# LingmaFuture/PRCV2025REID

Hardware: AMD Instinct MI355X
Metric: multimodal instances/sec (PxK, 5-modality) at 1/2/4/8 GPU; eval queries/sec (higher is better)
Workload: dtype bf16; 1 GPU; P=16,K=4 per GPU, vis/nir/sk/cp 224x224 + text (T<=77), CLIP ViT-B/16 + text tower random-init, MER-LoRA r=8, masks all-on, 400 ids, SDM+CE, fwd+bwd+grad sanitise/clip+AdamW (reference default trainable set); P=16, K=4, global_batch=64, lora_rank=8, accum_steps=1, parallelism=dp1

## Files before the change

### include/reid_hip.h

```cpp
#ifndef REID_HIP_H
#define REID_HIP_H

#include <stdint.h>

#ifdef __cplusplus
extern "C" {
#endif

typedef enum {
    REID_OK = 0,
    REID_ERR_ARG = -1,
    REID_ERR_LAUNCH = -2,
    REID_ERR_DEVICE = -3
} reid_status;

typedef enum { REID_BF16 = 0, REID_F32 = 1, REID_F16 = 2 } reid_dtype;

typedef enum {
    REID_ACT_NONE = 0,
    REID_ACT_GELU_ERF = 1,
    REID_ACT_QUICK_GELU = 2,
    REID_ACT_RELU = 3,
    REID_ACT_DGELU_ERF = 4,
    REID_ACT_DQUICK_GELU = 5,
// ... 45 lines not shown
                       const int32_t* row_index, const float* gamma, const float* mean, const float* rstd,
                       const void* dres, void* dx, int32_t dx_dtype, void* dx_bf16, int32_t lddx,
                       float* dgamma, float* dbeta, int32_t rows, int32_t cols,
                       const float* bf16_row_scale, int32_t rows_per_img, int32_t* overflow, void* stream);

int reid_patch_im2col(const float* images, void* patches, int32_t n_img, int32_t H, int32_t W,
                      int32_t patch, int32_t cin, void* stream);
int reid_cls_rows(const float* cls, const float* pos0, float* x, int32_t ldx, int32_t n_img,
                  int32_t tokens, int32_t cols, void* stream);

int reid_attn_fwd(const void* qkv, int32_t ld, const uint8_t* key_mask, void* out, int32_t ldo, float* lse,
                  int32_t n_seq, int32_t S, int32_t heads, int32_t causal, int32_t q_tiles, void* stream);
int reid_attn_bwd(const void* qkv, int32_t ld, const uint8_t* key_mask, const void* out, const void* dout,
                  int32_t ldo, const float* lse, void* dqkv, int32_t lddqkv, float* delta_ws,
                  int32_t n_seq, int32_t S, int32_t heads, int32_t causal, int32_t q_tiles, void* stream);

int reid_cast_f32_bf16(const float* src, void* dst, int64_t n, void* stream);
int reid_cast_bf16_f32(const void* src, float* dst, int64_t n, void* stream);
int reid_pack_bf16_table(const float* src, void* dst_bf16, const int64_t* table, int32_t n_entries, void* stream);
int reid_lora_bwd_fused(const void* dY, int32_t lddy, const void* T, int32_t ldt, const void* BT, int32_t ldbt, void* U, int32_t ldu,
                        float* dB, int32_t lddb, const int32_t* img_mod, int32_t rows_per_img, int32_t mask_r, int32_t M, int32_t N,
                        int32_t Rp, float scale, float* u_partial, int32_t u_mode, void* stream);
int reid_lora_da_fused(const void* X, int32_t ldx, const void* U, int32_t ldu, float* dA, int32_t ldda, const int32_t* img_mod,
                       int32_t rows_per_img, int32_t mask_r, int32_t M, int32_t K, int32_t Rp, int32_t n_groups, void* stream);

int reid_merge_lora_table(const int64_t* table, int32_t n_entries, int32_t max_tiles, const float* arena, void* weff,
                          int32_t Rp, int32_t r, int32_t nmod, float scaling, void* stream);
int reid_gather_rows_f32(const float* src, int32_t lds, const int32_t* index, float* dst, int32_t ldd,
                         int32_t rows, int32_t cols, void* stream);
int reid_embed_tokens(const float* tok, const float* pos, const int64_t* ids, float* out, int32_t B, int32_t T, int32_t D,
// ... 136 lines not shown
```

### prcv2025reid_amd/_lib.py

```python
import ctypes as C
import os

import torch

_HERE = os.path.dirname(os.path.abspath(__file__))
LIB_PATHS = {'bf16': os.path.join(_HERE, 'csrc', 'libreid_hip.so'), 'f16': os.path.join(_HERE, 'csrc', 'libreid_hip_f16.so')}
if os.environ.get('REID_LIB_BF16'):
    LIB_PATHS['bf16'] = os.environ['REID_LIB_BF16']
LIB_PATH = LIB_PATHS['bf16']
T16_DTYPES = {'bf16': torch.bfloat16, 'f16': torch.float16}
_flavor = os.environ.get('REID_T16', 'bf16')


def set_flavor(name: str):
    global _flavor
    if name not in LIB_PATHS:
        raise ValueError(f'unknown 16-bit flavor {name!r}')
    _flavor = name


def flavor() -> str:
    return _flavor


# ... 28 lines not shown
SIGNATURES = {
    'reid_last_error': (_S, []),
    'reid_version': (_I, []),
    'reid_flavor': (_I, []),
    'reid_check_device': (_I, [_I]),
    'reid_set_knob': (_I, [_S, _I]),
    'reid_mer_gemm': (_I, [_GEMM, _P]),
    'reid_gemm_tn': (_I, [_P, _P, _P, _I, _I, _I, _I, _I, _I, _F, _F, _P]),
    'reid_layernorm_fwd': (_I, [_P, _I, _P, _P, _P, _P, _P, _I, _P, _P, _I, _I, _F, _P]),
    'reid_add_layernorm_fwd': (_I, [_P, _I, _P, _I, _I, _P, _I, _P, _I, _P, _P, _P, _I, _P, _P, _I, _I, _F, _P]),
    'reid_layernorm_bwd': (_I, [_P, _I, _I, _P, _I, _P, _P, _P, _P, _P, _P, _I, _P, _I, _P, _P, _I, _I, _P, _I, _P, _P]),
    'reid_patch_im2col': (_I, [_P, _P, _I, _I, _I, _I, _I, _P]),
    'reid_cls_rows': (_I, [_P, _P, _P, _I, _I, _I, _I, _P]),
    'reid_attn_fwd': (_I, [_P, _I, _P, _P, _I, _P, _I, _I, _I, _I, _I, _P]),
    'reid_attn_bwd': (_I, [_P, _I, _P, _P, _P, _I, _P, _P, _I, _P, _I, _I, _I, _I, _I, _P]),
    'reid_cast_f32_bf16': (_I, [_P, _P, _I64, _P]),
    'reid_cast_bf16_f32': (_I, [_P, _P, _I64, _P]),
    'reid_pack_bf16_table': (_I, [_P, _P, _P, _I, _P]),
    'reid_lora_bwd_fused': (_I, [_P, _I, _P, _I, _P, _I, _P, _I, _P, _I, _P, _I, _I, _I, _I, _I, _F, _P, _I, _P]),
    'reid_lora_da_fused': (_I, [_P, _I, _P, _I, _P, _I, _P, _I, _I, _I, _I, _I, _I, _P]),
    'reid_merge_lora_table': (_I, [_P, _I, _I, _P, _P, _I, _I, _I, _F, _P]),
    'reid_gather_rows_f32': (_I, [_P, _I, _P, _P, _I, _I, _I, _P]),
    'reid_embed_tokens': (_I, [_P, _P, _P, _P, _I, _I, _I, _I, _P]),
    'reid_scatter_add_rows_f32': (_I, [_P, _I, _P, _P, _I, _I, _I, _I, _P]),
    'reid_bnneck_stats': (_I, [_P, _I, _I, _I, _P, _P, _P]),
    'reid_bnneck_fwd': (_I, [_P, _I, _P, _P, _P, _P, _P, _P, _F, _I, _P, _P, _I, _P, _P, _P, _I, _I, _F, _F, _F, _P]),
    'reid_bnneck_bwd_p1': (_I, [_P, _I, _P, _I, _P, _P, _P, _P, _P, _P, _P, _P, _I, _I, _F, _P]),
    'reid_bnneck_bwd_p2': (_I, [_P, _P, _I, _P, _P, _P, _P, _P, _F, _I, _P, _I, _I, _I, _P]),
    'reid_ce_ls_fwd': (_I, [_P, _I, _P, _P, _I, _I, _F, _P, _P, _P]),
    'reid_ce_ls_bwd': (_I, [_P, _I, _P, _P, _I, _I, _F, _P, _P, _I, _P]),
# ... 120 lines not shown
```

### prcv2025reid_amd/csrc/attention.hip

```cpp
#include "lds_tile.h"
#include <stdlib.h>

namespace {

using namespace ldstile;

constexpr float LOG2E = 1.4426950408889634f;

template <int NT>
__device__ __forceinline__ void stage_head(const bf16_t* __restrict__ base, int ld, int S, char* lds, int wave, int lane,
                                           int row_limit = 1 << 30) {
#pragma unroll
    for (int i = 0; i < 4; ++i) {
        const int rblk = (i * NT + wave) * 8;
        if (rblk >= row_limit) continue;
        stage_rows8(lds, rblk, lane, [&](int row, int c) { return base + (size_t)(row < S ? row : S - 1) * ld + c * 8; });
    }
}

__device__ __forceinline__ bf16x8 row_frag(const char* img, int row0, int kchunk, int lane) {
    const int row = row0 + (lane & 31);
    return *(const bf16x8*)(img + row * 128 + (swz(row, kchunk + (lane >> 5)) << 4));
}

// ... 42 lines not shown
__device__ __forceinline__ bf16x8 pack8(const f32x16& a, int s) {
    bf16x8 r;
#pragma unroll
    for (int j = 0; j < 8; ++j) r[j] = (short)f32_to_bf16(a[8 * s + j]);
    return r;
}

__device__ __forceinline__ int acc_row(int reg, int lane) { return (reg & 3) + 8 * (reg >> 2) + 4 * (lane >> 5); }

struct AttnParams {
    const bf16_t* qkv; int ld; const uint8_t* key_mask;
    bf16_t* out; int ldo; float* lse;
    const bf16_t* dout; bf16_t* dqkv; int lddqkv; float* delta;
    int n_seq, S, heads, causal;
    int q_tiles;
};

__device__ __forceinline__ void store_tile_row16(bf16_t* row, bool ok, const f32x16& t, float scale, int lane) {
#pragma unroll
    for (int j = 0; j < 2; ++j) {
        const int a = 8 * j, b = 8 * j + 4;
        const auto r0 = __builtin_amdgcn_permlane32_swap(pack_bf16x2(t[a] * scale, t[a + 1] * scale),
                                                         pack_bf16x2(t[b] * scale, t[b + 1] * scale), false, false);
        const auto r1 = __builtin_amdgcn_permlane32_swap(pack_bf16x2(t[a + 2] * scale, t[a + 3] * scale),
                                                         pack_bf16x2(t[b + 2] * scale, t[b + 3] * scale), false, false);
        if (ok) *(uint4*)(row + 8 * (2 * j + (lane >> 5))) = uint4{r0[0], r1[0], r0[1], r1[1]};
    }
}


template <int NT, bool TWO_PASS>
__global__ __launch_bounds__(NT * 64, TWO_PASS ? 4 : 1) void attn_fwd_kernel(const AttnParams p) {
    REID_T16_ENTER();
    extern __shared__ __attribute__((aligned(16))) char smem[];
    char* Ks = smem;
    char* Vs = smem + NT * 32 * 128;
    const int tid = threadIdx.x, lane = tid & 63;
    const int wave = __builtin_amdgcn_readfirstlane(tid >> 6);
    const int seq = blockIdx.x / p.heads, head = blockIdx.x % p.heads;
    const int d = p.heads * 64;
    const bf16_t* qb = p.qkv + (size_t)seq * p.S * p.ld + head * 64;
    stage_head<NT>(qb + d, p.ld, p.S, Ks, wave, lane);
    const int q0 = wave * 32;
    const int qi = q0 + (lane & 31);
    const int qrow = qi < p.S ? qi : p.S - 1;
    bf16x8 qf[4];
#pragma unroll
    for (int ks = 0; ks < 4; ++ks) qf[ks] = gfrag(qb, p.ld, qrow, 2 * ks, lane);
    stage_head<NT>(qb + 2 * d, p.ld, p.S, Vs, wave, lane);
    __syncthreads();
    if (q0 >= p.S || (p.q_tiles > 0 && wave >= p.q_tiles)) return;

    const FragOff fo = make_frag_off(lane);
    const uint8_t* km = p.key_mask ? p.key_mask + (size_t)seq * p.S : nullptr;
    const int h4 = 4 * (lane >> 5);
    const bool general = km != nullptr || p.causal;
    auto score_tile = [&](int kt) -> f32x16 {
        f32x16 t;
#pragma unroll
// ... 302 lines not shown
    char* Ds = smem + 2 * IMG;
    float* rowc = (float*)(Ds + NT * 32 * DS_ROW);
    const int tid = threadIdx.x, lane = tid & 63;
    const int wave = __builtin_amdgcn_readfirstlane(tid >> 6);
    const int seq = blockIdx.x / p.heads, head = blockIdx.x % p.heads;
    const int d = p.heads * 64;
    const bf16_t* qb = p.qkv + (size_t)seq * p.S * p.ld + head * 64;
    const bf16_t* gb = p.dout + (size_t)seq * p.S * p.ldo + head * 64;
    const bf16_t* ob = p.out + (size_t)seq * p.S * p.ldo + head * 64;
    const int nq = p.q_tiles > 0 ? (p.q_tiles < NT ? p.q_tiles : NT) : NT;
    const int q_rows = nq * 32;
    const int t0 = wave * 32;
    const int ti = t0 + (lane & 31);
    const int trow = ti < p.S ? ti : p.S - 1;
    const bool own_q = wave < nq;
    bf16x8 kf[4], vf[4];
#pragma unroll
    for (int ks = 0; ks < 4; ++ks) {
        kf[ks] = gfrag(qb + d, p.ld, trow, 2 * ks, lane);
        vf[ks] = gfrag(qb + 2 * d, p.ld, trow, 2 * ks, lane);
    }
    stage_head<NT>(qb, p.ld, p.S, Qs, wave, lane, q_rows);
    stage_head<NT>(gb, p.ldo, p.S, Gs, wave, lane, q_rows);
    bf16x8 of[4];
#pragma unroll
    for (int ks = 0; ks < 4; ++ks) of[ks] = gfrag(ob, p.ldo, trow, 2 * ks, lane);
    const size_t so = ((size_t)seq * p.heads + head) * p.S + trow;
    const float lse_v = p.lse[so];
    const FragOff fo = make_frag_off(lane);
    __syncthreads();
// ... 164 lines not shown
    (void)hipMemcpyToSymbol(HIP_SYMBOL(g_attn_bwd_trace), &ptr, sizeof(ptr));
}
#endif

#define DISPATCH_NT(nt, fn, ...)                \
    switch (nt) {                               \
        case 1: return fn<1>(__VA_ARGS__);      \
        case 2: return fn<2>(__VA_ARGS__);      \
        case 3: return fn<3>(__VA_ARGS__);      \
        case 4: return fn<4>(__VA_ARGS__);      \
        case 5: return fn<5>(__VA_ARGS__);      \
        case 6: return fn<6>(__VA_ARGS__);      \
        default: return fn<7>(__VA_ARGS__);     \
    }

extern "C" int reid_attn_fwd(const void* qkv, int32_t ld, const uint8_t* key_mask, void* out, int32_t ldo, float* lse,
                             int32_t n_seq, int32_t S, int32_t heads, int32_t causal, int32_t q_tiles, void* stream) {
    int rc = check_common("reid_attn_fwd", qkv, ld, n_seq, S, heads);
    if (rc) return rc;
    REID_CHECK_ARG(out && ldo >= heads * 64 && ldo % 4 == 0, "reid_attn_fwd: out/ldo");
    AttnParams p{(const bf16_t*)qkv, ld, key_mask, (bf16_t*)out, ldo, lse, nullptr, nullptr, 0, nullptr, n_seq, S, heads, causal, q_tiles};
    DISPATCH_NT((S + 31) / 32, launch_fwd, p, (hipStream_t)stream)
}

extern "C" int reid_attn_bwd(const void* qkv, int32_t ld, const uint8_t* key_mask, const void* out, const void* dout,
                             int32_t ldo, const float* lse, void* dqkv, int32_t lddqkv, float* delta_ws, int32_t n_seq,
                             int32_t S, int32_t heads, int32_t causal, int32_t q_tiles, void* stream) {
    int rc = check_common("reid_attn_bwd", qkv, ld, n_seq, S, heads);
    if (rc) return rc;
    REID_CHECK_ARG(out && dout && lse && dqkv && delta_ws, "reid_attn_bwd: null pointer");
    REID_CHECK_ARG(ldo >= heads * 64 && ldo % 8 == 0 && lddqkv >= 3 * heads * 64 && lddqkv % 4 == 0, "reid_attn_bwd: ldo/lddqkv");
    AttnParams p{(const bf16_t*)qkv, ld, key_mask, (bf16_t*)out, ldo, (float*)lse, (const bf16_t*)dout, (bf16_t*)dqkv, lddqkv,
                 delta_ws, n_seq, S, heads, causal, q_tiles};
    DISPATCH_NT((S + 31) / 32, launch_bwd, p, (hipStream_t)stream)
}
```

### prcv2025reid_amd/csrc/lora.hip

```cpp
#include "lds_tile.h"
#include <type_traits>

namespace {
using namespace ldstile;

constexpr int MT = 64;

__global__ __launch_bounds__(256) void merge_lora_kernel(const int64_t* __restrict__ table, const float* __restrict__ arena,
                                                         bf16_t* __restrict__ weff, int Rp, int r, int nmod, float s) {
    REID_T16_ENTER();
    const int64_t* e = table + (size_t)blockIdx.y * 8;
    const int N = (int)e[5], K = (int)e[6], G = (int)e[7];
    const int tiles_k = K / MT;
    if ((int)blockIdx.x >= (N / MT) * tiles_k) return;
    const float* __restrict__ W = (const float*)e[0];
    const float* __restrict__ A = arena + e[1];
    const float* __restrict__ B = arena + e[2];
    bf16_t* dst = weff + e[3];
    bf16_t* dstT = e[4] >= 0 ? weff + e[4] : nullptr;
    const int n0 = ((int)blockIdx.x / tiles_k) * MT, k0 = ((int)blockIdx.x % tiles_k) * MT;
    const int g = n0 / (N / G);
    const int R = nmod * r;
    __shared__ __attribute__((aligned(16))) float sW[MT][MT + 4];
    __shared__ __attribute__((aligned(16))) float sA[MT][MT + 4];
// ... 196 lines not shown

namespace image {
constexpr int N = fused::N, R = 32;
constexpr int ROW_BYTES = N * 2;
constexpr int IMG_BYTES = R * ROW_BYTES;
constexpr int NBUF = 3;
template <int RP> struct BwdGeo {
    static constexpr int T_BYTES = RP == 32 ? R * RP * 2 : R * 32;
    static constexpr int BUF_BYTES = IMG_BYTES + T_BYTES;
    static constexpr int USTAGE_BYTES = R * RP * 2;
    static constexpr int LDS_BYTES = NBUF * BUF_BYTES + USTAGE_BYTES;
};
using fused::Params;

constexpr int MAX_SPAN = 8;
__device__ __forceinline__ uint64_t span_mods(const int32_t* img_mod, int i0, int cnt) {
    uint64_t m = 0;
#pragma unroll
    for (int i = 0; i < MAX_SPAN; ++i) m |= (uint64_t)(img_mod[i0 + (i < cnt ? i : cnt - 1)] & 255) << (8 * i);
    return m;
}
__device__ __forceinline__ int span_mod(uint64_t mods, int i) { return (int)(mods >> (8 * i)) & 255; }

__device__ __forceinline__ bf16x8 tr_frag_swz(const char* img, int col0, int lane) {
    const int l16 = lane & 15, fq = lane >> 4;
    const int q = l16 >> 2, pp = l16 & 3;
    const int col = col0 + 4 * pp;
    const int r0 = 4 * fq + q, r1 = r0 + 16;
    const char* a0 = img + r0 * ROW_BYTES + (swz512(r0, col >> 3) << 4) + (col & 7) * 2;
    const char* a1 = img + r1 * ROW_BYTES + (swz512(r1, col >> 3) << 4) + (col & 7) * 2;
    return tr_join(tr_read(a0), tr_read(a1));
}

template <class P, class Run>
__device__ __forceinline__ void for_each_run(const P& p, Run run) {
    const int i0 = blockIdx.x * p.span, cnt = min(p.n_img - i0, p.span);
    const uint64_t mods = span_mods(p.img_mod, i0, cnt);
    for (int a = 0; a < cnt;) {
        const int mu = span_mod(mods, a);
        int b = a + 1;
        while (b < cnt && span_mod(mods, b) == mu) ++b;
        const int rbeg = (i0 + a) * p.rows_per_img;
        const int rend = min(p.M, (i0 + b) * p.rows_per_img);
        if (rbeg >= rend) break;
        a = b;
        run(rbeg, rend, mu, a < cnt);
    }
}

__device__ __forceinline__ void dma_tile(const bf16_t* const& src, const int& ld, const int& r0, const int& rend, const int& w, const int& lane, const uint32_t& base) {
#pragma unroll
    for (int j = 0; j < 6; ++j) {
        const int qd = w * 6 + j;
        const int g = qd * 64 + lane;
// ... 20 lines not shown
template <class Issue>
__device__ __forceinline__ int ring_refill(int t, int steps, int buf, Issue& issue) {
    const int nb = buf == 0 ? NBUF - 1 : buf - 1;
    if (t + 2 < steps) issue(t + 2, nb);
    return buf + 1 == NBUF ? 0 : buf + 1;
}

__global__ __launch_bounds__(256) void u_finish_kernel(const float* __restrict__ Up, bf16_t* __restrict__ U, int ldu, const int32_t* __restrict__ img_mod,
                                                       int rows_per_img, int mask_r, float scale, int M, int Rp) {
    REID_T16_ENTER();
    const int i = blockIdx.x * 256 + threadIdx.x;
    const int h = Rp >> 1;
    const int m = i / h, c = (i - m * h) * 2;
    if (m >= M) return;
    const int mu = img_mod[m / rows_per_img];
    const float a = Up[(size_t)m * Rp + c], b = Up[(size_t)m * Rp + c + 1];
    *(uint32_t*)(U + (size_t)m * ldu + c) = pack_bf16x2(c / mask_r == mu ? a * scale : 0.f, (c + 1) / mask_r == mu ? b * scale : 0.f);
}

template <int RP>
__device__ __forceinline__ void lora_bwd_image_run(const Params& p, char* smem, const int rbeg, const int rend, const int mu) {
    constexpr int BUF_BYTES = BwdGeo<RP>::BUF_BYTES;
    int tid = threadIdx.x;
    asm volatile("" : "+v"(tid));
    const int lane = tid & 63;
    const int w = __builtin_amdgcn_readfirstlane(tid >> 6);
    const int l16 = lane & 15, fq = lane >> 4;
    const int w0 = (mu * p.mask_r) & ~15;
    const int c_lo = mu * p.mask_r - w0, c_hi = c_lo + p.mask_r;
    const int steps = (rend - rbeg + R - 1) / R;
// ... 143 lines not shown
    __syncthreads();
    {
        const int rr = p.mask_r, total = N * rr;
        for (int idx = ftid; idx < total; idx += 512) {
            const int col = idx / rr, j = idx - col * rr;
            atomicAdd(p.dB + (size_t)col * p.lddb + mu * rr + j, fl[col * 16 + c_lo + j]);
        }
    }
}

template <int RP>
__global__ __launch_bounds__(512, 2) void lora_bwd_image_kernel(const Params p) {
    REID_T16_ENTER();
    static_assert(RP == 32 || RP == 64, "adapter columns");
    extern __shared__ __attribute__((aligned(16))) char smem[];
    for_each_run(p, [=](int rbeg, int rend, int mu, bool more) { lora_bwd_image_run<RP>(p, smem, rbeg, rend, mu); if (more) __syncthreads(); });
}

struct DaParams {
    const bf16_t* X; const bf16_t* U; float* dA;
    const int32_t* img_mod;
    int ldx, ldu, ldda, rows_per_img, mask_r, M, Rp, span, n_img;
};
template <int G>
__device__ __forceinline__ void lora_da_image_run(const DaParams& p, char* smem, const int rbeg, const int rend, const int mu, const bool more) {
    constexpr int UB = 4096;
    constexpr int BUF = IMG_BYTES + UB;
    const int tid = threadIdx.x, lane = tid & 63;
    const int w = __builtin_amdgcn_readfirstlane(tid >> 6);
    const int l16 = lane & 15, fq = lane >> 4;
    const int cblk = blockIdx.y;
// ... 47 lines not shown
    for (int e = 0; e < 4; ++e) {
        const int c = 4 * fq + e;
        if (c < c_lo || c >= c_hi) continue;
#pragma unroll
        for (int g = 0; g < G; ++g)
#pragma unroll
            for (int i = 0; i < 6; ++i)
                atomicAdd(p.dA + (size_t)(g * p.Rp + w0 + c) * p.ldda + (size_t)cblk * N + w * 96 + i * 16 + l16, acc[g][i][e]);
    }
}

template <int G>
__global__ __launch_bounds__(512, 2) void lora_da_image_kernel(const DaParams p) {
    REID_T16_ENTER();
    extern __shared__ __attribute__((aligned(16))) char smem[];
    for_each_run(p, [=](int rbeg, int rend, int mu, bool more) { lora_da_image_run<G>(p, smem, rbeg, rend, mu, more); });
}
}

}

static int lora_span(int n_img) {
    const int k = reid_knob(KNOB_LORA_SPAN);
    if (k == 1 || k == 2 || k == 4 || k == 8) return k;
    return n_img >= reid_num_cus() ? 4 : 1;
}

static bool lora_image_shape(int rows_per_img, int mask_r) { return rows_per_img >= image::R && mask_r <= 16 && 16 % mask_r == 0; }

extern "C" int reid_lora_bwd_fused(const void* dY, int32_t lddy, const void* T, int32_t ldt, const void* BT, int32_t ldbt, void* U,
                                   int32_t ldu, float* dB, int32_t lddb, const int32_t* img_mod, int32_t rows_per_img, int32_t mask_r,
// ... 76 lines not shown
```

### prcv2025reid_amd/engine.py

```python
from types import SimpleNamespace
from typing import Dict, List, Optional, Tuple

import math
import os

import torch

from . import _lib, ops

LIN = ('qkv', 'out', 'fc1', 'fc2')
REF_LIN = {'attn.q_proj': ('qkv', 0), 'attn.k_proj': ('qkv', 1), 'attn.v_proj': ('qkv', 2), 'attn.out_proj': ('out', 0),
           'mlp.fc1': ('fc1', 0), 'mlp.fc2': ('fc2', 0)}


def round_up(a, b):
    return (a + b - 1) // b * b


def grad_scale(amax):
    return torch.exp2(torch.floor(torch.log2(512.0 / amax))).clamp(2.0 ** -20, 2.0 ** 40)


class DenseGrads:

# ... 78 lines not shown
        e = self.ent[(l, nm)]
        n_out = e['N'] // e['G']
        return self.view_B(arena, l, nm)[g * n_out:(g + 1) * n_out, mu * r:(mu + 1) * r]

    def weff(self, arena, l, nm, transposed=False):
        e = self.ent[(l, nm)]
        N, K = e['N'], e['K']
        return self._view(arena, e['wET' if transposed else 'wE'], (self.nmod, K, N) if transposed else (self.nmod, N, K))

    def pk(self, pack, l, nm, which):
        e = self.ent[(l, nm)]
        G, K, N, Rp = e['G'], e['K'], e['N'], self.Rp
        return self._view(pack, e['p' + which], {'A': (G * Rp, K), 'AT': (K, G * Rp), 'B': (N, Rp), 'BT': (Rp, N)}[which])


class Engine:

    def __init__(self, arch: dict, P: Dict[str, torch.Tensor], lora_arena: torch.Tensor, device, layout: Optional[LoraLayout] = None):
        self.arch = arch
        self.P = P
        self.lora_arena = lora_arena
        self.dev = device
        self.lay = layout if layout is not None else LoraLayout(arch)
        self.S = (arch['image_size'] // arch['patch_size']) ** 2 + 1
        self.scaling = arch['lora_alpha'] / arch['lora_rank']
        self.flavor = _lib.flavor()
        self.loss_scaling = self.flavor == 'f16'
        self.dx_half = os.environ.get('REID_DX_HALF', '1') != '0'
        self.dx_overflow = torch.zeros(1, dtype=torch.int32, device=device)
        self._dense_ver = None
        self._lora_ver = None
        self._lora_pack = None
        self._weff = None
        self._merge_table = None
        self._table = None
        self._pack = self._text = self._side = None
        self._pack_event = None
        self._text_pending = None
        self._consts = {}
        self._rng = torch.Generator(device=device)
        self._rng.manual_seed(777)
        self.pending_drop_scales = None
        self._text_packed = None
        self.overlap_tn = os.environ.get('REID_TN_STREAM', '1') != '0'
# ... 109 lines not shown
        dv = sum(p._version for k, p in self.P.items() if k.startswith('clip_encoder.') and p is not self.lora_arena)
        tt = self.text_trains()
        dense_changed = dv != self._dense_ver or tt != self._text_packed
        if dense_changed:
            self.pack_dense(); self._dense_ver = dv; self._text_packed = tt
        lv = self.lora_arena._version
        if lv != self._lora_ver or dense_changed:
            self.pack_lora(); self._lora_ver = lv

    def drop_path_scales(self, n_img: int, rate: float):
        L = self.arch['vision_layers']
        keep = self._const(('dp_keep', L, float(rate)),
                           lambda: torch.tensor([1.0 - rate * l / max(1, L - 1) for l in range(L)], dtype=torch.float32))
        u = torch.rand(L, 2, n_img, device=self.dev, generator=self._rng)
        sc = torch.floor(u + keep.view(L, 1, 1)) / keep.view(L, 1, 1)
        return [(None, None) if rate * l / max(1, L - 1) <= 0.0 else (sc[l, 0], sc[l, 1]) for l in range(L)]

    def vision_forward(self, groups: List[Tuple[int, torch.Tensor]], save: bool, drop_scales=None):
        a, P, W, lay = self.arch, self.P, self.W, self.lay
        dev = self.dev
        S, d, ff, Rp = self.S, lay.d, lay.ff, lay.Rp
        heads = a['vision_heads']
        n_img = sum(g[1].shape[0] for g in groups)
        M = n_img * S
        ce = 'clip_encoder.'
        mods = []
        for mu, img in groups:
            mods += [mu] * img.shape[0]
        img_mod = self._const(('img_mod', tuple(mods)), lambda: torch.tensor(mods, dtype=torch.int32))
        f32, b16 = self._kw()
        x = torch.empty(M, d, **f32)
# ... 55 lines not shown

        L = a['vision_layers']
        nxt = None
        for l in range(L):
            lp = f'{ce}vision_layers.{l}.'
            if nxt is None:
                h = new('h', (M, d), b16); mean1 = new('m1', (M,), f32); rstd1 = new('r1', (M,), f32)
                ops.layernorm_fwd(x, P[lp + 'ln1.weight'], P[lp + 'ln1.bias'], y_bf16=h, mean=mean1, rstd=rstd1)
            else:
                h, mean1, rstd1 = nxt
                nxt = None
            qkv = new('qkv', (M, 3 * d), b16)
            ops.gemm(h, we(l, 'qkv'), qkv, bias=W[('v', l, 'bqkv')], row_groups=full.rg)
            last = l == L - 1
            o = new('o', (M, d), b16); lse = new('lse', (n_img, heads, S), f32)
            ops.attn_fwd(qkv, o, lse, n_img, S, heads, q_tiles=1 if last else 0)
            sa, sm_ = (None, None) if drop_scales is None else drop_scales[l]
            rows = cls if last else full
            xin, oin = (x.index_select(0, idxl), o.index_select(0, idxl)) if last else (x, o)
            Mr, rpi, rg = rows.M, rows.rpi, rows.rg
            xm = new('xm', (Mr, d), f32)
            h2 = new('h2', (Mr, d), b16); mean2 = new('m2', (Mr,), f32); rstd2 = new('r2', (Mr,), f32)
            if not last:
                yb = buf.get('yb')
                if yb is None:
                    yb = buf['yb'] = torch.empty(M, d, dtype=torch.float16, device=dev)
                ops.gemm(oin, we(l, 'out'), yb, bias=P[lp + 'attn.out_proj.shared_linear.bias'], row_groups=rg)
                ops.add_layernorm_fwd(xin, yb, xm, P[lp + 'ln2.weight'], P[lp + 'ln2.bias'], h2, mean2, rstd2, row_scale=sa, rows_per_img=rpi)
            else:
                ops.gemm(oin, we(l, 'out'), xm, bias=P[lp + 'attn.out_proj.shared_linear.bias'], R=xin, row_scale=sa, rows_per_img=rpi,
                         row_groups=rg)
                ops.layernorm_fwd(xm, P[lp + 'ln2.weight'], P[lp + 'ln2.bias'], y_bf16=h2, mean=mean2, rstd=rstd2)
# ... 14 lines not shown
                nxt = (new('h' + str((l + 1) & 1), (M, d), b16), new('m1' + str((l + 1) & 1), (M,), f32), new('r1' + str((l + 1) & 1), (M,), f32))
                ops.add_layernorm_fwd(xm, yb, xn, P[np_ + 'ln1.weight'], P[np_ + 'ln1.bias'], nxt[0], nxt[1], nxt[2], row_scale=sm_,
                                      rows_per_img=rpi)
            else:
                ops.gemm(g, we(l, 'fc2'), xn, bias=P[lp + 'mlp.fc2.shared_linear.bias'], R=xm, row_scale=sm_, rows_per_img=rpi,
                         row_groups=rg)
            if save:
                saved.append(dict(x=x, h=h, mean1=mean1, rstd1=rstd1, T=T, qkv=qkv, o=o, lse=lse, To=To, xm=xm, h2=h2,
                                  mean2=mean2, rstd2=rstd2, T1=T1, u=u, g=g, T2=T2, sa=sa, sm=sm_, cls=last, o_rows=oin))
            x = xn
        cls_h = torch.empty(n_img, d, **b16); mf = torch.empty(n_img, **f32); rf = torch.empty(n_img, **f32)
        ops.layernorm_fwd(x, P[ce + 'vision_ln_final.weight'], P[ce + 'vision_ln_final.bias'], y_bf16=cls_h, mean=mf, rstd=rf)
        feats = torch.empty(n_img, a['fusion_dim'], **f32)
        ops.gemm(cls_h, W['vproj'], feats)
        flush_lora_down()
        state = dict(layers=saved, x_final=x, idxl=idxl, mf=mf, rf=rf, n_img=n_img, cls_h=cls_h, groups=groups,
                     rows=(full, cls)) if save else None
        return feats, state

    def vision_dense_keys(self) -> List[str]:
        tp = 'clip_encoder.clip_model.'
        return [k for k in self.P if k.startswith('clip_encoder.') and not k.startswith(tp) and '.loras.' not in k
                and k != 'clip_encoder.text_proj.weight' and self.P[k] is not self.lora_arena]

    def vision_backward(self, st, dfeat: torch.Tensor, want_dense: bool = False):
        a, P, W, lay = self.arch, self.P, self.W, self.lay
        dev = self.dev
        S, d, ff, Rp, r = self.S, lay.d, lay.ff, lay.Rp, lay.r
        heads = a['vision_heads']
        n_img = st['n_img']; M = n_img * S
        ce = 'clip_encoder.'
        f32, b16 = self._kw()
# ... 27 lines not shown
        Uq = torch.empty(M, 3 * Rp, **b16)
        du2 = [torch.empty(M, ff, **b16) for _ in range(2)]
        dqkv2 = [torch.empty(M, 3 * d, **b16) for _ in range(2)]
        dxmb2 = [torch.empty(M, d, **b16) for _ in range(2)]
        dxb2 = [dxb, torch.empty(M, d, **b16)]
        dh = torch.empty(M, d, **b16); do = torch.empty(M, d, **b16)
        delta = torch.empty(n_img, heads, S, **f32)
        dxm = torch.empty(M, d, **gx)
        weT = lambda l, nm: lay.weff(self._weff, l, nm, transposed=True)
        main = torch.cuda.current_stream(dev)
        side = self._side_stream() if self.overlap_tn else None
        side_done = {}
        L = a['vision_layers']
        u_part = torch.empty(M, Rp, **f32)
        rows_full, rows_cls = st['rows']
        full = SimpleNamespace(**vars(rows_full), gy=dx, gyb=dxb2, U2=U2, U1=U1, Uo=Uo, du=du2, dh=dh, do=do, dxm=dxm, dxmb=dxmb2)
        cls = SimpleNamespace(**vars(rows_cls), gy=dx_c, gyb=[dxb_c] * 2,
                              U2=torch.empty(n_img, Rp, **b16), U1=torch.empty(n_img, Rp, **b16), Uo=torch.empty(n_img, Rp, **b16),
                              du=[torch.empty(n_img, ff, **b16)] * 2, dh=torch.empty(n_img, d, **b16), do=torch.empty(n_img, d, **b16),
                              dxm=torch.empty(n_img, d, **gx), dxmb=[torch.empty(n_img, d, **b16)] * 2)

        def adapter_grads(l, nm, dY, X, T, U, rows):
            if side is not None:
                wait_for(side, main)
            with torch.cuda.stream(side):
                BT, dB = pk(l, nm, 'BT'), lay.view_B(grad, l, nm)
                G = lay.ent[(l, nm)]['G']
                n = dY.shape[1] // G
                for g in range(G):
                    dYg, Tg, BTg, Ug, dBg = dY[:, g * n:(g + 1) * n], T[:, g * Rp:(g + 1) * Rp], BT[:, g * n:(g + 1) * n], \
                        U[:, g * Rp:(g + 1) * Rp], dB[g * n:(g + 1) * n]
                    if ops.lora_bwd_fused_ok(n, Rp, rows.rpi, r):
                        ops.lora_bwd_fused(dYg, Tg, BTg, Ug, dBg, rows.img_mod, rows.rpi, r, self.scaling,
                                           u_partial=u_part[:dY.shape[0]] if n > 768 else None)
                    else:
                        ops.gemm(dYg, BTg, Ug, **rows.mask)
                        ops.gemm_tn(dYg, Tg, dBg, beta=1.0)
                if ops.lora_da_fused_ok(X.shape[1], Rp, rows.rpi, r, G):
                    ops.lora_da_fused(X, U, lay.view_A(grad, l, nm), rows.img_mod, rows.rpi, r, n_groups=G)
                else:
                    ops.gemm_tn(U, X, lay.view_A(grad, l, nm), beta=1.0)

        for l in reversed(range(L)):
            s = st['layers'][l]
            lp = f'{ce}vision_layers.{l}.'
            b = l & 1
            c = s['cls']
            sc = cls if c else full
            gy, gyb, du, dxmb, rg = sc.gy, sc.gyb[b], sc.du[b], sc.dxmb[b], sc.rg
            dqkv = dqkv2[b]
            adapter_grads(l, 'fc2', gyb, s['g'], s['T2'], sc.U2, sc)
            ops.gemm(gyb, weT(l, 'fc2'), du, act='mul_aux', aux=s['u'], row_groups=rg)
            if want_dense:
                dense[lp + 'mlp.fc2.shared_linear.weight'] = dg.wgrad(gyb, s['g'])
# ... 2 lines not shown
            ops.gemm(du, weT(l, 'fc1'), sc.dh, row_groups=rg)
            if want_dense:
                dense[lp + 'mlp.fc1.shared_linear.weight'] = dg.wgrad(du, s['h2'])
                dense[lp + 'mlp.fc1.shared_linear.bias'] = dg.colsum(du)
            dg2, db2 = ln_pair(lp + 'ln2', d)
            ops.layernorm_bwd(sc.dh, s['xm'], P[lp + 'ln2.weight'], s['mean2'], s['rstd2'], sc.dxm, dx_bf16=dxmb, dres=gy,
                              bf16_row_scale=s['sa'], rows_per_img=sc.rpi, dgamma=dg2, dbeta=db2, overflow=ovf)
            adapter_grads(l, 'out', dxmb, s['o_rows'], s['To'], sc.Uo, sc)
            ops.gemm(dxmb, weT(l, 'out'), sc.do, row_groups=rg)
            if want_dense:
                dense[lp + 'attn.out_proj.shared_linear.weight'] = dg.wgrad(dxmb, s['o_rows'])
                dense[lp + 'attn.out_proj.shared_linear.bias'] = dg.colsum(dxmb)
            if c:
                do.zero_(); do.index_copy_(0, idxl, sc.do)
                dxm.zero_(); dxm.index_copy_(0, idxl, sc.dxm)
            ops.attn_bwd(s['qkv'], s['o'], do, s['lse'], dqkv, delta, n_img, S, heads, q_tiles=1 if c else 0)
            adapter_grads(l, 'qkv', dqkv, s['h'], s['T'], Uq, full)
            if side is not None:
                side_done[l] = side.record_event()
            if l == 0 and not want_dense:
                break
            ops.gemm(dqkv, weT(l, 'qkv'), dh, row_groups=full.rg)
            if want_dense:
                gw = dg.wgrad(dqkv, s['h']); gb_ = dg.colsum(dqkv)
                for gi, nm in enumerate('qkv'):
                    dense[lp + f'attn.{nm}_proj.shared_linear.weight'] = gw[gi * d:(gi + 1) * d]
                    dense[lp + f'attn.{nm}_proj.shared_linear.bias'] = gb_[gi * d:(gi + 1) * d]
            if l + 1 in side_done:
                main.wait_event(side_done.pop(l + 1))
            dg1, db1 = ln_pair(lp + 'ln1', d)
            ops.layernorm_bwd(dh, s['x'], P[lp + 'ln1.weight'], s['mean1'], s['rstd1'], dx, dx_bf16=dxb2[(l - 1) & 1], dres=dxm,
# ... 225 lines not shown
```

### prcv2025reid_amd/ops.py

```python
import ctypes as C
from typing import Optional

import torch

from . import _lib as L
from ._lib import BF16, F32, GemmArgs, check, lib, ptr, stream_ptr

ACT = {'none': L.ACT_NONE, 'gelu': L.ACT_GELU, 'quick_gelu': L.ACT_QUICK_GELU, 'relu': L.ACT_RELU,
       'dgelu': L.ACT_DGELU, 'dquick_gelu': L.ACT_DQUICK_GELU, 'drelu': L.ACT_DRELU,
       'mul_aux': L.ACT_MUL_AUX, 'gelu_dsave': L.ACT_GELU_DSAVE}


_gemm_profile = None
def gemm_profile_begin():
    global _gemm_profile
    _gemm_profile = []


def gemm_profile_end():
    global _gemm_profile
    p, _gemm_profile = _gemm_profile, None
    return p


# ... 109 lines not shown
        e1.record()
        nbytes = rows * x.shape[1] * ((2 if dy.dtype != torch.float32 else 4) + 4 + (dx.element_size() if dres is not None else 0) +
                                      dx.element_size() + (2 if dx_bf16 is not None else 0))
        _ln_profile.append((nbytes, e0, e1))


def patch_im2col(images, patches, patch, cin):
    n, _, H, W = images.shape
    check(lib().reid_patch_im2col(ptr(images), ptr(patches), n, H, W, patch, cin, stream_ptr()))


def cls_rows(cls, pos0, x, n_img, tokens):
    check(lib().reid_cls_rows(ptr(cls), ptr(pos0), ptr(x), x.stride(0), n_img, tokens, x.shape[1], stream_ptr()))


def attn_fwd(qkv, out, lse, n_seq, S, heads, causal=False, key_mask=None, q_tiles=0):
    check(lib().reid_attn_fwd(ptr(qkv), qkv.stride(0), ptr(key_mask), ptr(out), out.stride(0), ptr(lse), n_seq, S, heads,
                              int(causal), int(q_tiles), stream_ptr()))


def attn_bwd(qkv, out, dout, lse, dqkv, delta_ws, n_seq, S, heads, causal=False, key_mask=None, q_tiles=0):
    check(lib().reid_attn_bwd(ptr(qkv), qkv.stride(0), ptr(key_mask), ptr(out), ptr(dout), out.stride(0), ptr(lse),
                              ptr(dqkv), dqkv.stride(0), ptr(delta_ws), n_seq, S, heads, int(causal), int(q_tiles), stream_ptr()))


def cast_f32_bf16(src, dst):
    check(lib().reid_cast_f32_bf16(ptr(src), ptr(dst), src.numel(), stream_ptr()))
    return dst


def cast_bf16_f32(src, dst):
    check(lib().reid_cast_bf16_f32(ptr(src), ptr(dst), src.numel(), stream_ptr()))
    return dst


def lora_bwd_fused(dY, T, BT, U, dB, img_mod, rows_per_img, mask_r, scale, u_partial=None):
    N = dY.shape[1]
    nb = N // 768
# ... 370 lines not shown
```

Before: 2166 instances/s.

## Skip attention and LoRA backward work for drop-path-dropped images

```diff
diff --git a/include/reid_hip.h b/include/reid_hip.h
--- a/include/reid_hip.h
+++ b/include/reid_hip.h
@@ -83,6 +83,11 @@
 int reid_attn_bwd(const void* qkv, int32_t ld, const uint8_t* key_mask, const void* out, const void* dout,
                   int32_t ldo, const float* lse, void* dqkv, int32_t lddqkv, float* delta_ws,
                   int32_t n_seq, int32_t S, int32_t heads, int32_t causal, int32_t q_tiles, void* stream);
+int reid_attn_fwd_scaled(const void* qkv, int32_t ld, const uint8_t* key_mask, void* out, int32_t ldo, float* lse,
+                         int32_t n_seq, int32_t S, int32_t heads, int32_t causal, int32_t q_tiles, const float* seq_scale, void* stream);
+int reid_attn_bwd_scaled(const void* qkv, int32_t ld, const uint8_t* key_mask, const void* out, const void* dout,
+                         int32_t ldo, const float* lse, void* dqkv, int32_t lddqkv, float* delta_ws,
+                         int32_t n_seq, int32_t S, int32_t heads, int32_t causal, int32_t q_tiles, const float* seq_scale, void* stream);
 
 int reid_cast_f32_bf16(const float* src, void* dst, int64_t n, void* stream);
 int reid_cast_bf16_f32(const void* src, float* dst, int64_t n, void* stream);
diff --git a/prcv2025reid_amd/_lib.py b/prcv2025reid_amd/_lib.py
--- a/prcv2025reid_amd/_lib.py
+++ b/prcv2025reid_amd/_lib.py
@@ -66,6 +66,8 @@
     'reid_cls_rows': (_I, [_P, _P, _P, _I, _I, _I, _I, _P]),
     'reid_attn_fwd': (_I, [_P, _I, _P, _P, _I, _P, _I, _I, _I, _I, _I, _P]),
     'reid_attn_bwd': (_I, [_P, _I, _P, _P, _P, _I, _P, _P, _I, _P, _I, _I, _I, _I, _I, _P]),
+    'reid_attn_fwd_scaled': (_I, [_P, _I, _P, _P, _I, _P, _I, _I, _I, _I, _I, _P, _P]),
+    'reid_attn_bwd_scaled': (_I, [_P, _I, _P, _P, _P, _I, _P, _P, _I, _P, _I, _I, _I, _I, _I, _P, _P]),
     'reid_cast_f32_bf16': (_I, [_P, _P, _I64, _P]),
     'reid_cast_bf16_f32': (_I, [_P, _P, _I64, _P]),
     'reid_pack_bf16_table': (_I, [_P, _P, _P, _I, _P]),
diff --git a/prcv2025reid_amd/csrc/attention.hip b/prcv2025reid_amd/csrc/attention.hip
--- a/prcv2025reid_amd/csrc/attention.hip
+++ b/prcv2025reid_amd/csrc/attention.hip
@@ -80,7 +80,14 @@
     const bf16_t* dout; bf16_t* dqkv; int lddqkv; float* delta;
     int n_seq, S, heads, causal;
     int q_tiles;
+    const float* seq_scale;
 };
+
+__device__ __forceinline__ bool seq_skipped(const AttnParams& p, int seq) { return p.seq_scale != nullptr && p.seq_scale[seq] == 0.f; }
+__device__ __forceinline__ void zero_head_row(bf16_t* row, int lane) {
+#pragma unroll
+    for (int j = 0; j < 4; ++j) *(uint4*)(row + 16 * j + 8 * (lane >> 5)) = uint4{0u, 0u, 0u, 0u};
+}
 
 __device__ __forceinline__ void store_tile_row16(bf16_t* row, bool ok, const f32x16& t, float scale, int lane) {
 #pragma unroll
@@ -105,10 +112,17 @@
     const int wave = __builtin_amdgcn_readfirstlane(tid >> 6);
     const int seq = blockIdx.x / p.heads, head = blockIdx.x % p.heads;
     const int d = p.heads * 64;
+    const int q0 = wave * 32;
+    const int qi = q0 + (lane & 31);
+    if (seq_skipped(p, seq)) {
+        if (qi < p.S && !(p.q_tiles > 0 && wave >= p.q_tiles)) {
+            zero_head_row(p.out + ((size_t)seq * p.S + qi) * p.ldo + head * 64, lane);
+            if (p.lse && lane < 32) p.lse[((size_t)seq * p.heads + head) * p.S + qi] = 0.f;
+        }
+        return;
+    }
     const bf16_t* qb = p.qkv + (size_t)seq * p.S * p.ld + head * 64;
     stage_head<NT>(qb + d, p.ld, p.S, Ks, wave, lane);
-    const int q0 = wave * 32;
-    const int qi = q0 + (lane & 31);
     const int qrow = qi < p.S ? qi : p.S - 1;
     bf16x8 qf[4];
 #pragma unroll
@@ -441,6 +455,16 @@
     const int ti = t0 + (lane & 31);
     const int trow = ti < p.S ? ti : p.S - 1;
     const bool own_q = wave < nq;
+    if (seq_skipped(p, seq)) {
+        if (ti < p.S) {
+            bf16_t* zrow = p.dqkv + ((size_t)seq * p.S + ti) * p.lddqkv + head * 64;
+            zero_head_row(zrow, lane);
+            zero_head_row(zrow + d, lane);
+            zero_head_row(zrow + 2 * d, lane);
+            if (own_q && p.delta && lane < 32) p.delta[((size_t)seq * p.heads + head) * p.S + ti] = 0.f;
+        }
+        return;
+    }
     bf16x8 kf[4], vf[4];
 #pragma unroll
     for (int ks = 0; ks < 4; ++ks) {
@@ -635,23 +659,47 @@
         default: return fn<7>(__VA_ARGS__);     \
     }
 
-extern "C" int reid_attn_fwd(const void* qkv, int32_t ld, const uint8_t* key_mask, void* out, int32_t ldo, float* lse,
-                             int32_t n_seq, int32_t S, int32_t heads, int32_t causal, int32_t q_tiles, void* stream) {
+static int attn_fwd_launch(const void* qkv, int32_t ld, const uint8_t* key_mask, void* out, int32_t ldo, float* lse, int32_t n_seq, int32_t S,
+                           int32_t heads, int32_t causal, int32_t q_tiles, const float* seq_scale, void* stream) {
     int rc = check_common("reid_attn_fwd", qkv, ld, n_seq, S, heads);
     if (rc) return rc;
     REID_CHECK_ARG(out && ldo >= heads * 64 && ldo % 4 == 0, "reid_attn_fwd: out/ldo");
-    AttnParams p{(const bf16_t*)qkv, ld, key_mask, (bf16_t*)out, ldo, lse, nullptr, nullptr, 0, nullptr, n_seq, S, heads, causal, q_tiles};
+    AttnParams p{(const bf16_t*)qkv, ld, key_mask, (bf16_t*)out, ldo, lse, nullptr, nullptr, 0, nullptr, n_seq, S, heads, causal, q_tiles,
+                 (key_mask || causal) ? nullptr : seq_scale};
     DISPATCH_NT((S + 31) / 32, launch_fwd, p, (hipStream_t)stream)
 }
 
-extern "C" int reid_attn_bwd(const void* qkv, int32_t ld, const uint8_t* key_mask, const void* out, const void* dout,
-                             int32_t ldo, const float* lse, void* dqkv, int32_t lddqkv, float* delta_ws, int32_t n_seq,
-                             int32_t S, int32_t heads, int32_t causal, int32_t q_tiles, void* stream) {
+static int attn_bwd_launch(const void* qkv, int32_t ld, const uint8_t* key_mask, const void* out, const void* dout, int32_t ldo,
+                           const float* lse, void* dqkv, int32_t lddqkv, float* delta_ws, int32_t n_seq, int32_t S, int32_t heads,
+                           int32_t causal, int32_t q_tiles, const float* seq_scale, void* stream) {
     int rc = check_common("reid_attn_bwd", qkv, ld, n_seq, S, heads);
     if (rc) return rc;
     REID_CHECK_ARG(out && dout && lse && dqkv && delta_ws, "reid_attn_bwd: null pointer");
     REID_CHECK_ARG(ldo >= heads * 64 && ldo % 8 == 0 && lddqkv >= 3 * heads * 64 && lddqkv % 4 == 0, "reid_attn_bwd: ldo/lddqkv");
     AttnParams p{(const bf16_t*)qkv, ld, key_mask, (bf16_t*)out, ldo, (float*)lse, (const bf16_t*)dout, (bf16_t*)dqkv, lddqkv,
-                 delta_ws, n_seq, S, heads, causal, q_tiles};
+                 delta_ws, n_seq, S, heads, causal, q_tiles, (key_mask || causal) ? nullptr : seq_scale};
     DISPATCH_NT((S + 31) / 32, launch_bwd, p, (hipStream_t)stream)
 }
+
+extern "C" int reid_attn_fwd(const void* qkv, int32_t ld, const uint8_t* key_mask, void* out, int32_t ldo, float* lse,
+                             int32_t n_seq, int32_t S, int32_t heads, int32_t causal, int32_t q_tiles, void* stream) {
+    return attn_fwd_launch(qkv, ld, key_mask, out, ldo, lse, n_seq, S, heads, causal, q_tiles, nullptr, stream);
+}
+
+extern "C" int reid_attn_bwd(const void* qkv, int32_t ld, const uint8_t* key_mask, const void* out, const void* dout,
+                             int32_t ldo, const float* lse, void* dqkv, int32_t lddqkv, float* delta_ws, int32_t n_seq,
+                             int32_t S, int32_t heads, int32_t causal, int32_t q_tiles, void* stream) {
+    return attn_bwd_launch(qkv, ld, key_mask, out, dout, ldo, lse, dqkv, lddqkv, delta_ws, n_seq, S, heads, causal, q_tiles, nullptr, stream);
+}
+
+extern "C" int reid_attn_fwd_scaled(const void* qkv, int32_t ld, const uint8_t* key_mask, void* out, int32_t ldo, float* lse,
+                                    int32_t n_seq, int32_t S, int32_t heads, int32_t causal, int32_t q_tiles, const float* seq_scale,
+                                    void* stream) {
+    return attn_fwd_launch(qkv, ld, key_mask, out, ldo, lse, n_seq, S, heads, causal, q_tiles, seq_scale, stream);
+}
+
+extern "C" int reid_attn_bwd_scaled(const void* qkv, int32_t ld, const uint8_t* key_mask, const void* out, const void* dout,
+                                    int32_t ldo, const float* lse, void* dqkv, int32_t lddqkv, float* delta_ws, int32_t n_seq,
+                                    int32_t S, int32_t heads, int32_t causal, int32_t q_tiles, const float* seq_scale, void* stream) {
+    return attn_bwd_launch(qkv, ld, key_mask, out, dout, ldo, lse, dqkv, lddqkv, delta_ws, n_seq, S, heads, causal, q_tiles, seq_scale, stream);
+}
diff --git a/prcv2025reid_amd/csrc/lora.hip b/prcv2025reid_amd/csrc/lora.hip
--- a/prcv2025reid_amd/csrc/lora.hip
+++ b/prcv2025reid_amd/csrc/lora.hip
@@ -234,10 +234,14 @@
 using fused::Params;
 
 constexpr int MAX_SPAN = 8;
+constexpr int MOD_SKIP = 255;
 __device__ __forceinline__ uint64_t span_mods(const int32_t* img_mod, int i0, int cnt) {
     uint64_t m = 0;
 #pragma unroll
-    for (int i = 0; i < MAX_SPAN; ++i) m |= (uint64_t)(img_mod[i0 + (i < cnt ? i : cnt - 1)] & 255) << (8 * i);
+    for (int i = 0; i < MAX_SPAN; ++i) {
+        const int v = img_mod[i0 + (i < cnt ? i : cnt - 1)];
+        m |= (uint64_t)(v < 0 ? MOD_SKIP : v & 255) << (8 * i);
+    }
     return m;
 }
 __device__ __forceinline__ int span_mod(uint64_t mods, int i) { return (int)(mods >> (8 * i)) & 255; }
@@ -252,12 +256,17 @@
     return tr_join(tr_read(a0), tr_read(a1));
 }
 
-template <class P, class Run>
-__device__ __forceinline__ void for_each_run(const P& p, Run run) {
+template <class P, class Run, class Skip>
+__device__ __forceinline__ void for_each_run(const P& p, Run run, Skip skip) {
     const int i0 = blockIdx.x * p.span, cnt = min(p.n_img - i0, p.span);
     const uint64_t mods = span_mods(p.img_mod, i0, cnt);
     for (int a = 0; a < cnt;) {
         const int mu = span_mod(mods, a);
+        if (mu == MOD_SKIP) {
+            skip((i0 + a) * p.rows_per_img, min(p.M, (i0 + a + 1) * p.rows_per_img));
+            ++a;
+            continue;
+        }
         int b = a + 1;
         while (b < cnt && span_mod(mods, b) == mu) ++b;
         const int rbeg = (i0 + a) * p.rows_per_img;
@@ -308,6 +317,10 @@
     const int m = i / h, c = (i - m * h) * 2;
     if (m >= M) return;
     const int mu = img_mod[m / rows_per_img];
+    if (mu < 0) {
+        *(uint32_t*)(U + (size_t)m * ldu + c) = 0u;
+        return;
+    }
     const float a = Up[(size_t)m * Rp + c], b = Up[(size_t)m * Rp + c + 1];
     *(uint32_t*)(U + (size_t)m * ldu + c) = pack_bf16x2(c / mask_r == mu ? a * scale : 0.f, (c + 1) / mask_r == mu ? b * scale : 0.f);
 }
@@ -481,7 +494,14 @@
     REID_T16_ENTER();
     static_assert(RP == 32 || RP == 64, "adapter columns");
     extern __shared__ __attribute__((aligned(16))) char smem[];
-    for_each_run(p, [=](int rbeg, int rend, int mu, bool more) { lora_bwd_image_run<RP>(p, smem, rbeg, rend, mu); if (more) __syncthreads(); });
+    for_each_run(p, [=](int rbeg, int rend, int mu, bool more) { lora_bwd_image_run<RP>(p, smem, rbeg, rend, mu); if (more) __syncthreads(); },
+                 [=](int rbeg, int rend) {
+                     if (p.u_mode != 0) return;
+                     for (int i = threadIdx.x; i < (rend - rbeg) * (RP / 2); i += 512) {
+                         const int row = i / (RP / 2), c2 = i - row * (RP / 2);
+                         *(uint32_t*)(p.U + (size_t)(rbeg + row) * p.ldu + 2 * c2) = 0u;
+                     }
+                 });
 }
 
 struct DaParams {
@@ -559,7 +579,8 @@
 __global__ __launch_bounds__(512, 2) void lora_da_image_kernel(const DaParams p) {
     REID_T16_ENTER();
     extern __shared__ __attribute__((aligned(16))) char smem[];
-    for_each_run(p, [=](int rbeg, int rend, int mu, bool more) { lora_da_image_run<G>(p, smem, rbeg, rend, mu, more); });
+    for_each_run(p, [=](int rbeg, int rend, int mu, bool more) { lora_da_image_run<G>(p, smem, rbeg, rend, mu, more); },
+                 [](int, int) {});
 }
 }
 
diff --git a/prcv2025reid_amd/engine.py b/prcv2025reid_amd/engine.py
--- a/prcv2025reid_amd/engine.py
+++ b/prcv2025reid_amd/engine.py
@@ -116,6 +116,10 @@
         return self._view(pack, e['p' + which], {'A': (G * Rp, K), 'AT': (K, G * Rp), 'B': (N, Rp), 'BT': (Rp, N)}[which])
 
 
+class DropScales(list):
+    factors = None
+
+
 class Engine:
 
     def __init__(self, arch: dict, P: Dict[str, torch.Tensor], lora_arena: torch.Tensor, device, layout: Optional[LoraLayout] = None):
@@ -130,6 +134,7 @@
         self.loss_scaling = self.flavor == 'f16'
         self.dx_half = os.environ.get('REID_DX_HALF', '1') != '0'
         self.dx_overflow = torch.zeros(1, dtype=torch.int32, device=device)
+        self.dp_skip = int(os.environ.get('REID_DROPPATH_SKIP', '3'))
         self._dense_ver = None
         self._lora_ver = None
         self._lora_pack = None
@@ -269,7 +274,16 @@
                            lambda: torch.tensor([1.0 - rate * l / max(1, L - 1) for l in range(L)], dtype=torch.float32))
         u = torch.rand(L, 2, n_img, device=self.dev, generator=self._rng)
         sc = torch.floor(u + keep.view(L, 1, 1)) / keep.view(L, 1, 1)
-        return [(None, None) if rate * l / max(1, L - 1) <= 0.0 else (sc[l, 0], sc[l, 1]) for l in range(L)]
+        out = DropScales((None, None) if rate * l / max(1, L - 1) <= 0.0 else (sc[l, 0], sc[l, 1]) for l in range(L))
+        out.factors = sc
+        return out
+
+    def _skip_table(self, drop_scales, img_mod):
+        sc = getattr(drop_scales, 'factors', None)
+        if sc is None:
+            one = torch.ones(img_mod.numel(), dtype=torch.float32, device=self.dev)
+            sc = torch.stack([torch.stack([one if v is None else v.float() for v in pair]) for pair in drop_scales])
+        return torch.where(sc == 0, -1, img_mod)
 
     def vision_forward(self, groups: List[Tuple[int, torch.Tensor]], save: bool, drop_scales=None):
         a, P, W, lay = self.arch, self.P, self.W, self.lay
@@ -355,8 +369,8 @@
             ops.gemm(h, we(l, 'qkv'), qkv, bias=W[('v', l, 'bqkv')], row_groups=full.rg)
             last = l == L - 1
             o = new('o', (M, d), b16); lse = new('lse', (n_img, heads, S), f32)
-            ops.attn_fwd(qkv, o, lse, n_img, S, heads, q_tiles=1 if last else 0)
             sa, sm_ = (None, None) if drop_scales is None else drop_scales[l]
+            ops.attn_fwd(qkv, o, lse, n_img, S, heads, q_tiles=1 if last else 0, seq_scale=sa if self.dp_skip & 1 else None)
             rows = cls if last else full
             xin, oin = (x.index_select(0, idxl), o.index_select(0, idxl)) if last else (x, o)
             Mr, rpi, rg = rows.M, rows.rpi, rows.rg
@@ -401,8 +415,9 @@
         feats = torch.empty(n_img, a['fusion_dim'], **f32)
         ops.gemm(cls_h, W['vproj'], feats)
         flush_lora_down()
+        skip_mod = self._skip_table(drop_scales, img_mod) if (save and drop_scales is not None and self.dp_skip & 2) else None
         state = dict(layers=saved, x_final=x, idxl=idxl, mf=mf, rf=rf, n_img=n_img, cls_h=cls_h, groups=groups,
-                     rows=(full, cls)) if save else None
+                     rows=(full, cls), skip_mod=skip_mod) if save else None
         return feats, state
 
     def vision_dense_keys(self) -> List[str]:
@@ -460,6 +475,7 @@
         L = a['vision_layers']
         u_part = torch.empty(M, Rp, **f32)
         rows_full, rows_cls = st['rows']
+        skip_mod = st.get('skip_mod')
         full = SimpleNamespace(**vars(rows_full), gy=dx, gyb=dxb2, U2=U2, U1=U1, Uo=Uo, du=du2, dh=dh, do=do, dxm=dxm, dxmb=dxmb2)
         cls = SimpleNamespace(**vars(rows_cls), gy=dx_c, gyb=[dxb_c] * 2,
                               U2=torch.empty(n_img, Rp, **b16), U1=torch.empty(n_img, Rp, **b16), Uo=torch.empty(n_img, Rp, **b16),
@@ -469,6 +485,9 @@
         def adapter_grads(l, nm, dY, X, T, U, rows):
             if side is not None:
                 wait_for(side, main)
+            imod = rows.img_mod
+            if skip_mod is not None and rows.rpi == S:
+                imod = skip_mod[l, 0 if nm in ('qkv', 'out') else 1]
             with torch.cuda.stream(side):
                 BT, dB = pk(l, nm, 'BT'), lay.view_B(grad, l, nm)
                 G = lay.ent[(l, nm)]['G']
@@ -477,13 +496,13 @@
                     dYg, Tg, BTg, Ug, dBg = dY[:, g * n:(g + 1) * n], T[:, g * Rp:(g + 1) * Rp], BT[:, g * n:(g + 1) * n], \
                         U[:, g * Rp:(g + 1) * Rp], dB[g * n:(g + 1) * n]
                     if ops.lora_bwd_fused_ok(n, Rp, rows.rpi, r):
-                        ops.lora_bwd_fused(dYg, Tg, BTg, Ug, dBg, rows.img_mod, rows.rpi, r, self.scaling,
+                        ops.lora_bwd_fused(dYg, Tg, BTg, Ug, dBg, imod, rows.rpi, r, self.scaling,
                                            u_partial=u_part[:dY.shape[0]] if n > 768 else None)
                     else:
                         ops.gemm(dYg, BTg, Ug, **rows.mask)
                         ops.gemm_tn(dYg, Tg, dBg, beta=1.0)
                 if ops.lora_da_fused_ok(X.shape[1], Rp, rows.rpi, r, G):
-                    ops.lora_da_fused(X, U, lay.view_A(grad, l, nm), rows.img_mod, rows.rpi, r, n_groups=G)
+                    ops.lora_da_fused(X, U, lay.view_A(grad, l, nm), imod, rows.rpi, r, n_groups=G)
                 else:
                     ops.gemm_tn(U, X, lay.view_A(grad, l, nm), beta=1.0)
 
@@ -516,7 +535,8 @@
             if c:
                 do.zero_(); do.index_copy_(0, idxl, sc.do)
                 dxm.zero_(); dxm.index_copy_(0, idxl, sc.dxm)
-            ops.attn_bwd(s['qkv'], s['o'], do, s['lse'], dqkv, delta, n_img, S, heads, q_tiles=1 if c else 0)
+            ops.attn_bwd(s['qkv'], s['o'], do, s['lse'], dqkv, delta, n_img, S, heads, q_tiles=1 if c else 0,
+                         seq_scale=s['sa'] if self.dp_skip & 1 else None)
             adapter_grads(l, 'qkv', dqkv, s['h'], s['T'], Uq, full)
             if side is not None:
                 side_done[l] = side.record_event()
diff --git a/prcv2025reid_amd/ops.py b/prcv2025reid_amd/ops.py
--- a/prcv2025reid_amd/ops.py
+++ b/prcv2025reid_amd/ops.py
@@ -147,14 +147,21 @@
     check(lib().reid_cls_rows(ptr(cls), ptr(pos0), ptr(x), x.stride(0), n_img, tokens, x.shape[1], stream_ptr()))
 
 
-def attn_fwd(qkv, out, lse, n_seq, S, heads, causal=False, key_mask=None, q_tiles=0):
-    check(lib().reid_attn_fwd(ptr(qkv), qkv.stride(0), ptr(key_mask), ptr(out), out.stride(0), ptr(lse), n_seq, S, heads,
-                              int(causal), int(q_tiles), stream_ptr()))
-
-
-def attn_bwd(qkv, out, dout, lse, dqkv, delta_ws, n_seq, S, heads, causal=False, key_mask=None, q_tiles=0):
-    check(lib().reid_attn_bwd(ptr(qkv), qkv.stride(0), ptr(key_mask), ptr(out), ptr(dout), out.stride(0), ptr(lse),
-                              ptr(dqkv), dqkv.stride(0), ptr(delta_ws), n_seq, S, heads, int(causal), int(q_tiles), stream_ptr()))
+def _seq_scale(seq_scale, n_seq):
+    if seq_scale is not None and (seq_scale.dtype != torch.float32 or seq_scale.numel() != n_seq or not seq_scale.is_contiguous()):
+        raise ValueError(f'seq_scale must be a contiguous fp32 [{n_seq}] tensor')
+    return ptr(seq_scale)
+
+
+def attn_fwd(qkv, out, lse, n_seq, S, heads, causal=False, key_mask=None, q_tiles=0, seq_scale=None):
+    check(lib().reid_attn_fwd_scaled(ptr(qkv), qkv.stride(0), ptr(key_mask), ptr(out), out.stride(0), ptr(lse), n_seq, S, heads,
+                                     int(causal), int(q_tiles), _seq_scale(seq_scale, n_seq), stream_ptr()))
+
+
+def attn_bwd(qkv, out, dout, lse, dqkv, delta_ws, n_seq, S, heads, causal=False, key_mask=None, q_tiles=0, seq_scale=None):
+    check(lib().reid_attn_bwd_scaled(ptr(qkv), qkv.stride(0), ptr(key_mask), ptr(out), ptr(dout), out.stride(0), ptr(lse),
+                                     ptr(dqkv), dqkv.stride(0), ptr(delta_ws), n_seq, S, heads, int(causal), int(q_tiles),
+                                     _seq_scale(seq_scale, n_seq), stream_ptr()))
 
 
 def cast_f32_bf16(src, dst):
```

Result: no change. 2182 instances/s (median of 6 runs) (+0.7%).
